# althonos/pyhmmer

Hardware: AMD Instinct MI355X
Metric: GCUPS (DP cells/s) + seqs/s for hmmsearch, Pfam-A vs proteome, 1/2/4/8 GPUs (higher is better)
Workload: dtype u8/i16 filters (MSV, Viterbi), f32 Forward/Backward

## Files before the change

pyhmmer_amd/csrc/p7x_msv.hip:

```cpp
#include <cstdlib>
#include <iterator>
#include "p7x_device.hpp"
#include "p7x_kernels.hpp"
#include "p7x_launch.hpp"

namespace p7x {

typedef short s2 __attribute__((ext_vector_type(2)));

__device__ __forceinline__ s2 as_s2(uint32_t u) { return __builtin_bit_cast(s2, u); }
__device__ __forceinline__ uint32_t as_u32(s2 v) { return __builtin_bit_cast(uint32_t, v); }
__device__ __forceinline__ s2 pk_max(s2 a, s2 b) { return __builtin_elementwise_max(a, b); }
__device__ __forceinline__ s2 pk_adds(s2 a, s2 b) { return __builtin_elementwise_add_sat(a, b); }
__device__ __forceinline__ s2 pk_subs(s2 a, s2 b) { return __builtin_elementwise_sub_sat(a, b); }
__device__ __forceinline__ s2 splat(int v) { s2 r; r.x = (short) v; r.y = (short) v; return r; }
__device__ __forceinline__ s2 swap_halves(s2 v) { return as_s2(__builtin_amdgcn_alignbit(as_u32(v), as_u32(v), 16)); }

typedef _Float16 h2 __attribute__((ext_vector_type(2)));
__device__ __forceinline__ h2 as_h2(s2 v) { return __builtin_bit_cast(h2, v); }
__device__ __forceinline__ s2 as_s2(h2 v) { return __builtin_bit_cast(s2, v); }
__device__ __forceinline__ s2 h_adds(s2 a, s2 b)
{
  const h2 z = { (_Float16) 0.0f, (_Float16) 0.0f }, o = { (_Float16) 1.0f, (_Float16) 1.0f };
  return as_s2(__builtin_elementwise_min(__builtin_elementwise_max(as_h2(a) + as_h2(b), z), o));
}
__device__ __forceinline__ s2 h_subs(s2 a, s2 b)
{
  const h2 z = { (_Float16) 0.0f, (_Float16) 0.0f }, o = { (_Float16) 1.0f, (_Float16) 1.0f };
  return as_s2(__builtin_elementwise_min(__builtin_elementwise_max(as_h2(a) - as_h2(b), z), o));
}
__device__ __forceinline__ s2 h_max(s2 a, s2 b) { return as_s2(__builtin_elementwise_maximum(as_h2(a), as_h2(b))); }
__device__ __forceinline__ s2 h_max3(s2 a, s2 b, s2 c)
{ return as_s2(__builtin_elementwise_maximum(__builtin_elementwise_maximum(as_h2(a), as_h2(b)), as_h2(c))); }
__device__ __forceinline__ s2 h_splat(int units)
{ const _Float16 x = (_Float16) ((float) units * (1.0f / 256.0f)); h2 r; r.x = x; r.y = x; return as_s2(r); }
__device__ __forceinline__ uint32_t h_of_i16_pair(uint32_t w)
{
  const int lo = max((int) (short) (w & 0xffffu), -512), hi = max((int) (short) (w >> 16), -512);
  return __builtin_bit_cast(uint32_t, __builtin_amdgcn_cvt_pkrtz((float) lo * (1.0f / 256.0f), (float) hi * (1.0f / 256.0f)));
}


constexpr int msv_stride_c(int R)
{
  int S = R + (R & 1);
  if (((S / 2) & 1) == 0) S += 2;
  return S;
}
constexpr int msv_lane_stride_c(int R, int K)
{
  if (K == 1) return msv_stride_c(R);
  int s = R + (R & 1);
  while (s % 64 != 2) s += 2;
  return s;
}
constexpr int msv_row_stride_c(int R, int K) { return K * msv_lane_stride_c(R, K); }
constexpr bool msv_uniform_c(int K) { return K >= 8; }
constexpr int msv_parities_c(int K) { return msv_uniform_c(K) ? 1 : 2; }
constexpr int msv_even_imm_c(int R, int K) { return K == 1 ? kTabRows * msv_row_stride_c(R, K) * 4 : 0; }
constexpr int msv_even_add_c(int R, int K) { return (K == 1 || msv_uniform_c(K)) ? 0 : kTabRows * msv_row_stride_c(R, K) * 4; }
constexpr int msv_block_c(int K) { return K == 1 ? 256 : 512; }
template <int K, bool H = false> __device__ __forceinline__ s2 target_max(s2 m)
{
  auto mx = [](s2 a, s2 b) { if constexpr (H) return h_max(a, b); else return pk_max(a, b); };
  if constexpr (K >= 2) m = mx(m, as_s2((uint32_t) __builtin_amdgcn_update_dpp(0, (int) as_u32(m), 0xB1, 0xf, 0xf, false)));
  if constexpr (K >= 4) m = mx(m, as_s2((uint32_t) __builtin_amdgcn_update_dpp(0, (int) as_u32(m), 0x4E, 0xf, 0xf, false)));
  if constexpr (K >= 8) m = mx(m, as_s2((uint32_t) __builtin_amdgcn_update_dpp(0, (int) as_u32(m), 0x141, 0xf, 0xf, false)));
  return m;
}
template <int K> __device__ __forceinline__ s2 carry_in(s2 last, s2 edge, int h)
{
  if constexpr (K == 1) return edge;
  const s2 up = as_s2((uint32_t) __builtin_amdgcn_update_dpp(0, (int) as_u32(last), 0x111, 0xf, 0xf, false));
  return h == 0 ? edge : up;
}

struct Chunk { uint2 e0, e1, e2, e3; };

template <int OFF>
__device__ __forceinline__ void lds_issue4(uint32_t addr, Chunk &c)
{
  asm volatile("ds_read_b64 %0, %4 offset:%5\n\t"
               "ds_read_b64 %1, %4 offset:%6\n\t"
               "ds_read_b64 %2, %4 offset:%7\n\t"
               "ds_read_b64 %3, %4 offset:%8"
               : "=&v"(c.e0), "=&v"(c.e1), "=&v"(c.e2), "=&v"(c.e3)
               : "v"(addr), "i"(OFF), "i"(OFF + 8), "i"(OFF + 16), "i"(OFF + 24));
}
template <int OFF>
__device__ __forceinline__ void lds_issue2(uint32_t addr, Chunk &c)
{
  asm volatile("ds_read_b64 %0, %2 offset:%3\n\t"
               "ds_read_b64 %1, %2 offset:%4"
               : "=&v"(c.e0), "=&v"(c.e1)
               : "v"(addr), "i"(OFF), "i"(OFF + 8));
}
template <int PENDING>
__device__ __forceinline__ void lds_wait4(Chunk &c)
{
  asm volatile("s_waitcnt lgkmcnt(%4)" : "+v"(c.e0), "+v"(c.e1), "+v"(c.e2), "+v"(c.e3) : "i"(PENDING));
}
template <int PENDING>
__device__ __forceinline__ void lds_wait2(Chunk &c)
{
  asm volatile("s_waitcnt lgkmcnt(%2)" : "+v"(c.e0), "+v"(c.e1) : "i"(PENDING));
}

template <int R, int TB, bool ODD, int T, int FAST = 0, bool U = false>
struct RowChunks {
  static_assert(!U || ODD, "the uniform row reads the register below: it is walked from the top register down");
  static_assert(R % 4 == 0, "a row is walked in chunks of 8 registers and a last one of 4: the register count must be a multiple of 4");
  static constexpr int NT = (R + 7) / 8;
  static constexpr int TBASE = TB;
  static constexpr int pairs(int t) { return (t == NT - 1 && (R % 8) != 0) ? 2 : 4; }

  template <int TT>
  static __device__ __forceinline__ void issue(uint32_t addr, Chunk &c)
  {
    if constexpr (pairs(TT) == 4) lds_issue4<TBASE + TT * 32>(addr, c); else lds_issue2<TBASE + TT * 32>(addr, c);
  }

  template <int JJ>
  static __device__ __forceinline__ void pair(s2 (&v)[R], const uint2 e, const s2 xB, const s2 carry, s2 &accA, s2 &accB)
  {
    if constexpr (U) {
      s2 pred = carry;
      if constexpr (JJ > 0) pred = v[2 * JJ - 1];
      const s2 d1 = as_s2(__builtin_amdgcn_alignbit(as_u32(v[2 * JJ + 1]), as_u32(v[2 * JJ]), 16));
      const s2 d0 = as_s2(__builtin_amdgcn_alignbit(as_u32(v[2 * JJ]), as_u32(pred), 16));
      if constexpr (FAST == 2) {
        v[2 * JJ + 1] = h_adds(d1, as_s2(e.y));
        v[2 * JJ] = h_adds(d0, as_s2(e.x));
        if constexpr (JJ & 1) { accB = h_max3(accB, v[2 * JJ], v[2 * JJ + 1]); asm volatile("" : "+v"(accB)); }
        else { accA = h_max3(accA, v[2 * JJ], v[2 * JJ + 1]); asm volatile("" : "+v"(accA)); }
      } else if constexpr (FAST == 1) {
        v[2 * JJ + 1] = pk_adds(d1, as_s2(e.y));
        v[2 * JJ] = pk_adds(d0, as_s2(e.x));
        accA = pk_max(accA, v[2 * JJ]);
        accB = pk_max(accB, v[2 * JJ + 1]);
        asm volatile("" : "+v"(accA), "+v"(accB));
      } else {
        v[2 * JJ + 1] = pk_max(d1, xB) + as_s2(e.y);
        accA = pk_max(accA, v[2 * JJ + 1]);
        v[2 * JJ] = pk_max(d0, xB) + as_s2(e.x);
        accB = pk_max(accB, v[2 * JJ]);
      }
    } else if constexpr (FAST == 2) {
      if constexpr (ODD) {
        v[2 * JJ + 1] = h_adds(v[2 * JJ], as_s2(e.y));
        s2 pred = carry;
        if constexpr (JJ > 0) pred = v[2 * JJ - 1];
        v[2 * JJ] = h_adds(pred, as_s2(e.x));
      } else {
        v[2 * JJ] = h_adds(v[2 * JJ], as_s2(e.x));
        v[2 * JJ + 1] = h_adds(v[2 * JJ + 1], as_s2(e.y));
      }
      if constexpr (JJ & 1) { accB = h_max3(accB, v[2 * JJ], v[2 * JJ + 1]); asm volatile("" : "+v"(accB)); }
      else { accA = h_max3(accA, v[2 * JJ], v[2 * JJ + 1]); asm volatile("" : "+v"(accA)); }
    } else if constexpr (FAST == 1) {
      if constexpr (ODD) {
        v[2 * JJ + 1] = pk_adds(v[2 * JJ], as_s2(e.y));
        s2 pred = carry;
        if constexpr (JJ > 0) pred = v[2 * JJ - 1];
        v[2 * JJ] = pk_adds(pred, as_s2(e.x));
      } else {
        v[2 * JJ] = pk_adds(v[2 * JJ], as_s2(e.x));
        v[2 * JJ + 1] = pk_adds(v[2 * JJ + 1], as_s2(e.y));
      }
      accA = pk_max(accA, v[2 * JJ]);
      accB = pk_max(accB, v[2 * JJ + 1]);
      asm volatile("" : "+v"(accA), "+v"(accB));
    } else if constexpr (ODD) {
      const s2 t1 = pk_max(v[2 * JJ], xB);
      v[2 * JJ + 1] = t1 + as_s2(e.y);
      accA = pk_max(accA, v[2 * JJ + 1]);
      s2 t0 = pk_max(carry, xB);
      if constexpr (JJ > 0) t0 = pk_max(v[2 * JJ - 1], xB);
      v[2 * JJ] = t0 + as_s2(e.x);
      accB = pk_max(accB, v[2 * JJ]);
    } else {
      v[2 * JJ] = pk_max(v[2 * JJ], xB) + as_s2(e.x);
      accA = pk_max(accA, v[2 * JJ]);
      v[2 * JJ + 1] = pk_max(v[2 * JJ + 1], xB) + as_s2(e.y);
      accB = pk_max(accB, v[2 * JJ + 1]);
    }
  }

  static __device__ __forceinline__ void run(s2 (&v)[R], uint32_t addr, Chunk &cur, Chunk &nxt, const s2 xB, const s2 carry, s2 &accA, s2 &accB)
  {
    constexpr bool last = ODD ? (T == 0) : (T == NT - 1);
    constexpr int TN = ODD ? T - 1 : T + 1;
    constexpr int np = pairs(T);
    if constexpr (!last) {
      issue<TN>(addr, nxt);
      if constexpr (np == 4) lds_wait4<pairs(TN)>(cur); else lds_wait2<pairs(TN)>(cur);
    } else {
      if constexpr (np == 4) lds_wait4<0>(cur); else lds_wait2<0>(cur);
    }
    if constexpr (ODD) {
      if constexpr (np == 4) {
        pair<4 * T + 3>(v, cur.e3, xB, carry, accA, accB);
        pair<4 * T + 2>(v, cur.e2, xB, carry, accA, accB);
      }
      pair<4 * T + 1>(v, cur.e1, xB, carry, accA, accB);
      pair<4 * T + 0>(v, cur.e0, xB, carry, accA, accB);
    } else {
      pair<4 * T + 0>(v, cur.e0, xB, carry, accA, accB);
      pair<4 * T + 1>(v, cur.e1, xB, carry, accA, accB);
      if constexpr (np == 4) {
        pair<4 * T + 2>(v, cur.e2, xB, carry, accA, accB);
        pair<4 * T + 3>(v, cur.e3, xB, carry, accA, accB);
      }
    }
    if constexpr (!last) RowChunks<R, TB, ODD, TN, FAST, U>::run(v, addr, nxt, cur, xB, carry, accA, accB);
  }
};

template <int R, int K, bool ODD>
__device__ __forceinline__ void msv_row(s2 (&v)[R], uint32_t addr, int h, s2 &xB, s2 &xJ, s2 &xEmax,
                                        const s2 basev, const s2 tecv, const s2 tjbmv, const s2 zerov)
{
  constexpr int NT = (R + 7) / 8;
  constexpr bool U = msv_uniform_c(K), DOWN = ODD || U;
  constexpr int T0 = DOWN ? NT - 1 : 0;
  constexpr int TB = DOWN ? 0 : msv_even_imm_c(R, K);
  const s2 carry = DOWN ? carry_in<K>(v[R - 1], xB, h) : xB;
  Chunk ca, cb;
  RowChunks<R, TB, DOWN, T0, 0, U>::template issue<T0>(addr, ca);
  s2 accA = splat(kNegPad), accB = accA;
  RowChunks<R, TB, DOWN, T0, 0, U>::run(v, addr, ca, cb, xB, carry, accA, accB);
  s2 m = pk_max(accA, accB);
  m = pk_max(m, swap_halves(m));
  m = target_max<K>(m);
  xEmax = pk_max(xEmax, m);
  m = m - tecv;
  xJ = pk_max(xJ, m);
  xB = pk_max(pk_max(basev, xJ) - tjbmv, zerov);
}

template <int K> struct MsvItem {
  int g, t, h;
  __device__ __forceinline__ MsvItem(int group, int part, int lane) : g(group), t(part * (64 / K) + lane / K), h(lane % K) {}
};

template <int R, int K>
__global__ void __launch_bounds__(msv_block_c(K)) msv_kernel(const ArgRef ref)
{
  extern __shared__ __attribute__((aligned(16))) uint32_t lds[];
  constexpr int S = msv_row_stride_c(R, K), Rs = msv_lane_stride_c(R, K), BLK = msv_block_c(K);
  const MsvArgs a = load_args<MsvArgs>(ref);
  const int nitems = (a.group_list ? *a.group_count : a.ngroups - a.group_first) * K;
  if (nitems <= 0 || *a.counter >= nitems) return;
  {
    constexpr int n4 = (msv_parities_c(K) * kTabRows * S) / 4;
    const uint4 *src = reinterpret_cast<const uint4 *>(a.tab);
    uint4 *dst = reinterpret_cast<uint4 *>(lds);
    for (int i = threadIdx.x; i < n4; i += BLK) dst[i] = src[i];
  }
  __syncthreads();

  const int lane = threadIdx.x & 63;
  const s2 basev = splat(a.base), tecv = splat(a.tec), zerov = splat(0);

  for (;;) {
    int item = 0;
    if (lane == 0) item = atomicAdd(a.counter, 1);
    item = __builtin_amdgcn_readfirstlane(item);
    if (item >= nitems) break;
    const int gi = item / K;
    const MsvItem<K> it(a.group_list ? __builtin_amdgcn_readfirstlane(a.group_list[gi]) : gi + a.group_first, item % K, lane);

    const int slot = it.g * 64 + it.t;
    const int L = a.slot_len[slot];
    const int nblk = a.grp_nblk[it.g];
    const uint4 *tp = a.tiles + a.grp_off[it.g] + it.t;
    const s2 tjbmv = splat((int) a.tjb_tab[L] + a.tbm);
    const uint32_t lane_col = (uint32_t) it.h * (uint32_t) (Rs * 4);

    s2 v[R];
#pragma unroll
    for (int j = 0; j < R; ++j) v[j] = zerov;
    s2 xJ = zerov, xEmax = zerov;
    s2 xB = pk_max(basev - tjbmv, zerov);

    uint4 cur = tp[0];
    for (int b = 0; b < nblk; ++b) {
      const uint4 nxt = (b + 1 < nblk) ? tp[(size_t) (b + 1) * 64] : cur;
      uint32_t w0 = cur.x, w1 = cur.y, w2 = cur.z, w3 = cur.w;
#pragma unroll 1
      for (int c = 0; c < 8; ++c) {
        const uint32_t x0 = w0 & 0xffu, x1 = (w0 >> 8) & 0xffu;
        w0 = __builtin_amdgcn_alignbit(w1, w0, 16); w1 = __builtin_amdgcn_alignbit(w2, w1, 16);
        w2 = __builtin_amdgcn_alignbit(w3, w2, 16); w3 >>= 16;
        msv_row<R, K, true >(v, x0 * (uint32_t) (S * 4) + lane_col, it.h, xB, xJ, xEmax, basev, tecv, tjbmv, zerov);
        msv_row<R, K, false>(v, x1 * (uint32_t) (S * 4) + lane_col + (uint32_t) msv_even_add_c(R, K), it.h, xB, xJ, xEmax, basev, tecv, tjbmv, zerov);
      }
      cur = nxt;
    }
    if (L > 0 && it.h == 0) {
      const int xe = xEmax.x;
      a.out_xJ[slot] = (xe >= 255 - a.bias) ? (int16_t) -1 : (int16_t) xJ.x;
    }
  }
}

template <int R, int K, bool H>
__device__ __forceinline__ void msv_fast_body(const MsvArgs &a, uint32_t *lds)
{
  constexpr int S = msv_row_stride_c(R, K), Rs = msv_lane_stride_c(R, K), BLK = msv_block_c(K);
  constexpr int MODE = H ? 2 : 1;
  const int nitems = (a.ngroups - a.group_first) * K;
  if (*a.counter >= nitems) return;
  {
    constexpr int n4 = (msv_parities_c(K) * kTabRows * S) / 4;
    const uint4 *src = reinterpret_cast<const uint4 *>(a.tab);
    uint4 *dst = reinterpret_cast<uint4 *>(lds);
    for (int i = threadIdx.x; i < n4; i += BLK) {
      uint4 w = src[i];
      if constexpr (H) { w.x = h_of_i16_pair(w.x); w.y = h_of_i16_pair(w.y); w.z = h_of_i16_pair(w.z); w.w = h_of_i16_pair(w.w); }
      dst[i] = w;
    }
  }
  __syncthreads();

  const int lane = threadIdx.x & 63;
  const s2 floorv = H ? as_s2(0u) : splat(-32768);
  constexpr int NT = (R + 7) / 8;
  auto mx = [](s2 x, s2 y) { if constexpr (H) return h_max(x, y); else return pk_max(x, y); };

  for (;;) {
    int item = 0;
    if (lane == 0) item = atomicAdd(a.counter, 1);
    item = __builtin_amdgcn_readfirstlane(item);
    if (item >= nitems) break;
    const MsvItem<K> it(item / K + a.group_first, item % K, lane);

    const int slot = it.g * 64 + it.t;
    const int L = a.slot_len[slot];
    const int nblk = a.grp_nblk[it.g];
    const uint2 *tp = reinterpret_cast<const uint2 *>(a.tiles + a.grp_off[it.g] + it.t);
    const int tjbm = (int) a.tjb_tab[L] + a.tbm;
    const uint32_t lane_col = (uint32_t) it.h * (uint32_t) (Rs * 4);

    s2 v[R];
#pragma unroll
    for (int j = 0; j < R; ++j) v[j] = floorv;
    int xJ = 0, xEmax = 0;
    int xB = max(a.base - tjbm, 0);
    const int F0 = xB - a.tec;
    const s2 Tv = H ? h_splat(tjbm + a.tec) : splat(tjbm + a.tec - 32768);
    s2 accA = floorv, accB = floorv;
    auto fold = [&](const s2 m2) -> int {
      int rel;
      if constexpr (H) { const h2 m = as_h2(m2); rel = (int) (256.0f * fmaxf((float) m.x, (float) m.y)); }
      else rel = max((int) m2.x, (int) m2.y) + 32768;
      const int xE = rel + xB;
      xEmax = max(xEmax, xE);
      xJ = max(xJ, xE - a.tec);
      return max(max(a.base, xJ) - tjbm, 0);
    };

    uint2 cur = tp[0];
    for (int hb = 0; hb < 2 * nblk; ++hb) {
      const uint2 nxt = (hb + 1 < 2 * nblk) ? tp[(size_t) ((hb + 1) >> 1) * 128 + ((hb + 1) & 1)] : cur;
      uint32_t w0 = cur.x, w1 = cur.y;
#pragma unroll 1
      for (int c = 0; c < 4; ++c) {
        const uint32_t x0 = w0 & 0xffu, x1 = (w0 >> 8) & 0xffu;
        w0 = __builtin_amdgcn_alignbit(w1, w0, 16); w1 >>= 16;
#pragma unroll
        for (int half = 0; half < 2; ++half) {
          Chunk ca, cb;
          if constexpr (msv_uniform_c(K)) {
            const uint32_t addr = (half == 0 ? x0 : x1) * (uint32_t) (S * 4) + lane_col;
            const s2 carry = carry_in<K>(v[R - 1], floorv, it.h);
            RowChunks<R, 0, true, NT - 1, MODE, true>::template issue<NT - 1>(addr, ca);
            RowChunks<R, 0, true, NT - 1, MODE, true>::run(v, addr, ca, cb, floorv, carry, accA, accB);
          } else if (half == 0) {
            const uint32_t addr = x0 * (uint32_t) (S * 4) + lane_col;
            const s2 carry = carry_in<K>(v[R - 1], floorv, it.h);
            RowChunks<R, 0, true, NT - 1, MODE>::template issue<NT - 1>(addr, ca);
            RowChunks<R, 0, true, NT - 1, MODE>::run(v, addr, ca, cb, floorv, carry, accA, accB);
          } else {
            const uint32_t addr = x1 * (uint32_t) (S * 4) + lane_col + (uint32_t) msv_even_add_c(R, K);
            RowChunks<R, msv_even_imm_c(R, K), false, 0, MODE>::template issue<0>(addr, ca);
            RowChunks<R, msv_even_imm_c(R, K), false, 0, MODE>::run(v, addr, ca, cb, floorv, floorv, accA, accB);
          }
          const s2 m2 = target_max<K, H>(mx(accA, accB));
          if (__builtin_expect(__any(as_u32(mx(m2, Tv)) != as_u32(Tv)), 0)) {
            asm volatile("; re-bias: the begin score moved" ::: "memory");
            const int xBn = fold(m2);
            const s2 dv = H ? h_splat(xBn - xB) : splat(xBn - xB);
#pragma unroll
            for (int j = 0; j < R; ++j) v[j] = H ? h_subs(v[j], dv) : pk_subs(v[j], dv);
            xB = xBn;
            accA = floorv; accB = floorv;
          }
        }
      }
      cur = nxt;
    }
    fold(target_max<K, H>(mx(accA, accB)));
    const bool ambiguous = (L > 0) && (xJ == F0) && !(xEmax >= 255 - a.bias);
    if (L > 0 && it.h == 0) a.out_xJ[slot] = (xEmax >= 255 - a.bias) ? (int16_t) -1 : (int16_t) xJ;
    if (__any(ambiguous) && lane == 0) { const int idx = atomicAdd(a.amb_count, 1); a.amb_groups[idx] = it.g; }
  }
}

constexpr int msv_min_blocks_c(int R, int K) { return K > 1 ? 2 : (R <= 92 ? 4 : (R <= 136 ? 3 : 2)); }

template <int R, int K, bool H>
__global__ void __launch_bounds__(msv_block_c(K), msv_min_blocks_c(R, K)) msv_fast_kernel(const ArgRef ref)
{
  extern __shared__ __attribute__((aligned(16))) uint32_t lds[];
  const MsvArgs a = load_args<MsvArgs>(ref);
  msv_fast_body<R, K, H>(a, lds);
}

#define P7X_TILES_TIER0(X) X(8, 1) X(12, 1) X(16, 1) X(20, 1) X(24, 1) X(28, 1) X(32, 1) X(36, 1) X(40, 1) X(44, 1) X(48, 1) X(52, 1) \
                           X(56, 1) X(60, 1) X(64, 1) X(68, 1) X(72, 1) X(76, 1) X(80, 1) X(84, 1) X(88, 1) X(92, 1)
#define P7X_TILES_TIER1(X) X(96, 1) X(100, 1) X(104, 1) X(108, 1) X(112, 1) X(116, 1) X(120, 1) X(124, 1) X(128, 1) X(132, 1) X(136, 1)
#define P7X_TILES_TIER2(X) X(140, 1) X(144, 1) X(148, 1) X(152, 1) X(156, 1) X(160, 1) X(176, 1) X(192, 1) X(208, 1) X(224, 1)
#define P7X_TILES_TIER3(X) X(120, 2) X(128, 2) X(136, 2) X(144, 2) X(152, 2) X(160, 2) X(168, 2) X(176, 2) X(184, 2) X(192, 2) X(200, 2) \
                           X(208, 2) X(216, 2) X(224, 2)
#define P7X_TILES_TIER4(X) X(120, 4) X(128, 4)
#define P7X_TILES_TIER5(X) X(64, 8) X(72, 8) X(80, 8) X(88, 8) X(96, 8) X(104, 8) X(112, 8) X(120, 8) X(128, 8)
constexpr int msv_tier_block_c(int T) { return T <= 2 ? 256 : 512; }
constexpr int msv_tier_min_blocks_c(int T) { return T == 0 ? 4 : (T == 1 ? 3 : 2); }

template <int TIER>
__global__ void __launch_bounds__(msv_tier_block_c(TIER), msv_tier_min_blocks_c(TIER)) msv_tier_kernel(const ArgRef ref)
{
  extern __shared__ __attribute__((aligned(16))) uint32_t lds[];
  const MsvArgs a = load_args<MsvArgs>(ref);
  const int R = __builtin_amdgcn_readfirstlane(a.R);
#define P7X_TILE(r, k) case r: msv_fast_body<r, k, true>(a, lds); break;
  if constexpr (TIER == 0) { switch (R) { P7X_TILES_TIER0(P7X_TILE) default: break; } }
  else if constexpr (TIER == 1) { switch (R) { P7X_TILES_TIER1(P7X_TILE) default: break; } }
  else if constexpr (TIER == 2) { switch (R) { P7X_TILES_TIER2(P7X_TILE) default: break; } }
  else if constexpr (TIER == 3) { switch (R) { P7X_TILES_TIER3(P7X_TILE) default: break; } }
  else if constexpr (TIER == 4) { switch (R) { P7X_TILES_TIER4(P7X_TILE) default: break; } }
  else { switch (R) { P7X_TILES_TIER5(P7X_TILE) default: break; } }
#undef P7X_TILE
}


#define P7X_R_ONLY(r, k) r,
static const int kRList[] = { P7X_TILES_TIER0(P7X_R_ONLY) P7X_TILES_TIER1(P7X_R_ONLY) P7X_TILES_TIER2(P7X_R_ONLY) };
static const int kRList2[] = { P7X_TILES_TIER3(P7X_R_ONLY) };
static const int kRList4[] = { P7X_TILES_TIER4(P7X_R_ONLY) };
static const int kRList8[] = { P7X_TILES_TIER5(P7X_R_ONLY) };
#undef P7X_R_ONLY
static bool msv_tile_exists(int R, int K)
{
  auto in = [R](const int *b, const int *e) { for (; b != e; ++b) if (*b == R) return true; return false; };
  switch (K) {
    case 1: return in(std::begin(kRList), std::end(kRList));
    case 2: return in(std::begin(kRList2), std::end(kRList2));
    case 4: return in(std::begin(kRList4), std::end(kRList4));
    case 8: return in(std::begin(kRList8), std::end(kRList8));
    default: return false;
  }
}

int msv_pick(int M, int *K)
{
  const int need = (M + 1) / 2 + 1;
  *K = 1;
  for (int r : kRList) if (r >= need) return r;
  *K = 2;
  for (int r : kRList2) if (2 * r >= need) return r;
  *K = 4;
  for (int r : kRList4) if (4 * r >= need) return r;
  *K = 8;
  if (debug_opt(OPT_MSV_K8) != 0)
    for (int r : kRList8) if (8 * r >= (M + 1) / 2) return r;
  *K = 0;
  return -1;
}

static int row_stride(int R, int K)
{
  int rs = R + (R & 1);
  if (K == 1) { if (((rs / 2) & 1) == 0) rs += 2; return rs; }
  while (rs % 64 != 2) rs += 2;
  return K * rs;
}
int msv_stride(int R, int K) { return row_stride(R, K); }
int msv_table_dwords(int R, int K) { return msv_parities_c(K) * kTabRows * row_stride(R, K); }

void msv_build_tables(const Profile &p, int R, int K, std::vector<uint32_t> &out)
{
  const int S = row_stride(R, K), Rs = S / K;
  out.assign((size_t) msv_table_dwords(R, K), 0);
  auto sval = [&](int x, int k) -> int {
    if (x >= p.Kp || k < 1 || k > p.M) return kNegPad;
    return (int) p.bias_b - (int) p.rb[(size_t) x * (p.M + 1) + k];
  };
  auto pack = [](int lo, int hi) -> uint32_t { return ((uint32_t) (uint16_t) (int16_t) lo) | ((uint32_t) (uint16_t) (int16_t) hi << 16); };
  if (msv_uniform_c(K)) {
    for (int x = 0; x < kTabRows; ++x)
      for (int h = 0; h < K; ++h)
        for (int r = 0; r < Rs; ++r) {
          const int j = h * R + r;
          out[(size_t) x * S + (size_t) h * Rs + r] = r < R ? pack(sval(x, 2 * j + 1), sval(x, 2 * j + 2)) : pack(kNegPad, kNegPad);
        }
    return;
  }
  for (int x = 0; x < kTabRows; ++x)
    for (int h = 0; h < K; ++h)
      for (int r = 0; r < Rs; ++r) {
        const bool live = r < R;
        const int j = h * R + r;
        out[((size_t) 0 * kTabRows + x) * S + (size_t) h * Rs + r] = live ? pack(sval(x, 2 * j - 1), sval(x, 2 * j)) : pack(kNegPad, kNegPad);
        out[((size_t) 1 * kTabRows + x) * S + (size_t) h * Rs + r] = live ? pack(sval(x, 2 * j), sval(x, 2 * j + 1)) : pack(kNegPad, kNegPad);
      }
}

template <int R, int K>
static int launch_RK(const ArgRun<MsvArgs> &main, const ArgRun<MsvArgs> *amb, int num_cu, hipStream_t st, bool amb_only = false)
{
  constexpr int BLK = msv_block_c(K);
  const size_t lds_bytes = (size_t) msv_parities_c(K) * kTabRows * msv_row_stride_c(R, K) * 4;
  int per_cu_exact = 0, per_cu_fast = 0, per_cu_half = 0;
  int pst = kernel_blocks_per_cu(&msv_kernel<R, K>, BLK, lds_bytes, &per_cu_exact);
  if (pst == P7X_OK) pst = kernel_blocks_per_cu(&msv_fast_kernel<R, K, false>, BLK, lds_bytes, &per_cu_fast);
  if (pst == P7X_OK) pst = kernel_blocks_per_cu(&msv_fast_kernel<R, K, true>, BLK, lds_bytes, &per_cu_half);
  if (pst != P7X_OK) return pst;
  if (amb_only) {
    hipLaunchKernelGGL((msv_kernel<R, K>), dim3(lane_grid(32, 32, amb->n), (unsigned) amb->n), dim3(BLK), lds_bytes, st, amb->ref());
    P7X_HIP(hipGetLastError());
    return P7X_OK;
  }
  constexpr int wpb = BLK / 64;
  long want = 1;
  for (int i = 0; i < main.n; ++i) want = std::max<long>(want, ((long) (main.at(i).ngroups - main.at(i).group_first) * K + wpb - 1) / wpb);
  if (amb == nullptr) {
    const unsigned gx = lane_grid_pull(want, (long) num_cu * per_cu_exact, main.n, debug_opt(OPT_MSV_LANE_BLOCKS) == 0);
    hipLaunchKernelGGL((msv_kernel<R, K>), dim3(gx, (unsigned) main.n), dim3(BLK), lds_bytes, st, main.ref());
    P7X_HIP(hipGetLastError());
    return P7X_OK;
  }
  const bool half = debug_opt(OPT_MSV_F16) != 0;
  int per_cu2 = half ? per_cu_half : per_cu_fast;
  const int cap = debug_opt(OPT_MSV_BLOCKS_PER_CU);
  if (cap > 0 && per_cu2 > cap) per_cu2 = cap;
  const unsigned gx2 = lane_grid_pull(want, (long) num_cu * per_cu2, main.n, debug_opt(OPT_MSV_LANE_BLOCKS) == 0);
  if (half) hipLaunchKernelGGL((msv_fast_kernel<R, K, true>), dim3(gx2, (unsigned) main.n), dim3(BLK), lds_bytes, st, main.ref());
  else hipLaunchKernelGGL((msv_fast_kernel<R, K, false>), dim3(gx2, (unsigned) main.n), dim3(BLK), lds_bytes, st, main.ref());
  P7X_HIP(hipGetLastError());
  hipLaunchKernelGGL((msv_kernel<R, K>), dim3(lane_grid(32, 32, amb->n), (unsigned) amb->n), dim3(BLK), lds_bytes, st, amb->ref());
  P7X_HIP(hipGetLastError());
  return P7X_OK;
}

static int msv_launch_impl(int R, int K, const ArgRun<MsvArgs> &main, const ArgRun<MsvArgs> *amb, int num_cu, hipStream_t st, bool amb_only);

int msv_launch(int R, int K, const ArgRun<MsvArgs> &main, const ArgRun<MsvArgs> *amb, int num_cu, hipStream_t st)
{ return msv_launch_impl(R, K, main, amb, num_cu, st, false); }

int msv_exact_launch(int R, int K, const ArgRun<MsvArgs> &amb, int num_cu, hipStream_t st)
{ return msv_launch_impl(R, K, amb, &amb, num_cu, st, true); }

int msv_tier(int R, int K)
{
  if (K == 1) return R <= 92 ? 0 : (R <= 136 ? 1 : 2);
  return K == 2 ? 3 : (K == 4 ? 4 : 5);
}

template <int TIER>
static int launch_tier(const ArgRun<MsvArgs> &main, int num_cu, hipStream_t st)
{
  constexpr int BLK = msv_tier_block_c(TIER), K = TIER <= 2 ? 1 : (TIER == 3 ? 2 : (TIER == 4 ? 4 : 8));
  int Rmax = 0;
  long want = 1;
  constexpr int wpb = BLK / 64;
  for (int i = 0; i < main.n; ++i) {
    const MsvArgs &a = main.at(i);
    if (msv_tier(a.R, K) != TIER || !msv_tile_exists(a.R, K)) { set_error("msv_tier_launch: a lane of another tier, or a register tile without a kernel"); return P7X_EINVAL; }
    Rmax = std::max(Rmax, a.R);
    want = std::max<long>(want, ((long) (a.ngroups - a.group_first) * K + wpb - 1) / wpb);
  }
  const size_t lds_bytes = (size_t) msv_table_dwords(Rmax, K) * 4;
  constexpr int Rtop = TIER == 0 ? 92 : (TIER == 1 ? 136 : (TIER >= 4 ? 128 : 224));
  int per_cu = 0;
  const int pst = kernel_blocks_per_cu(&msv_tier_kernel<TIER>, BLK, lds_bytes, &per_cu, (size_t) msv_table_dwords(Rtop, K) * 4);
  if (pst != P7X_OK) return pst;
  const unsigned gx = lane_grid_pull(want, (long) num_cu * per_cu, main.n, debug_opt(OPT_MSV_LANE_BLOCKS) == 0);
  hipLaunchKernelGGL((msv_tier_kernel<TIER>), dim3(gx, (unsigned) main.n), dim3(BLK), lds_bytes, st, main.ref());
  P7X_HIP(hipGetLastError());
  return P7X_OK;
}

int msv_tier_launch(int tier, const ArgRun<MsvArgs> &main, int num_cu, hipStream_t st)
{
  if (main.n <= 0) return P7X_OK;
  switch (tier) {
    case 0: return launch_tier<0>(main, num_cu, st);
    case 1: return launch_tier<1>(main, num_cu, st);
    case 2: return launch_tier<2>(main, num_cu, st);
    case 3: return launch_tier<3>(main, num_cu, st);
    case 4: return launch_tier<4>(main, num_cu, st);
    case 5: return launch_tier<5>(main, num_cu, st);
    default: set_error("msv_tier_launch: no such tier"); return P7X_EINVAL;
  }
}

static int msv_launch_impl(int R, int K, const ArgRun<MsvArgs> &main, const ArgRun<MsvArgs> *amb, int num_cu, hipStream_t st, bool amb_only)
{
  if (main.n <= 0) return P7X_OK;
  switch (K * 1000 + R) {
#define P7X_CASE(r, k) case k * 1000 + r: return launch_RK<r, k>(main, amb, num_cu, st, amb_only);
    P7X_TILES_TIER0(P7X_CASE) P7X_TILES_TIER1(P7X_CASE) P7X_TILES_TIER2(P7X_CASE) P7X_TILES_TIER3(P7X_CASE) P7X_TILES_TIER4(P7X_CASE) P7X_TILES_TIER5(P7X_CASE)
#undef P7X_CASE
    default: set_error("msv_launch: unsupported register tile"); return P7X_EINVAL;
  }
}

}
```

Before: 27100.

## Prefetch next residue row's LDS scores and trim MSV loop to wave max length

Issues the LDS loads for the second residue's first score chunk while the first residue's last chunk is still being consumed, so the two residue rows overlap instead of draining the queue between them. The per-group block loop is also bounded by the longest sequence in the wave rather than the group's padded block count, which skips padded residues. The register-pinning asm hints in the fp16 path now target the other accumulator. The read-ahead raises register pressure and adds chunk-buffer swapping logic, so it is limited to R <= 208.

```diff
diff --git a/pyhmmer_amd/csrc/p7x_msv.hip b/pyhmmer_amd/csrc/p7x_msv.hip
--- a/pyhmmer_amd/csrc/p7x_msv.hip
+++ b/pyhmmer_amd/csrc/p7x_msv.hip
@@ -3,6 +3,7 @@
 #include "p7x_device.hpp"
 #include "p7x_kernels.hpp"
 #include "p7x_launch.hpp"
+#include "p7x_wave.hpp"
 
 namespace p7x {
 
@@ -41,6 +42,7 @@
 }
 
 
+constexpr bool msv_read_ahead_c(int R) { return R <= 208; }
 constexpr int msv_stride_c(int R)
 {
   int S = R + (R & 1);
@@ -131,8 +133,8 @@
       if constexpr (FAST == 2) {
         v[2 * JJ + 1] = h_adds(d1, as_s2(e.y));
         v[2 * JJ] = h_adds(d0, as_s2(e.x));
-        if constexpr (JJ & 1) { accB = h_max3(accB, v[2 * JJ], v[2 * JJ + 1]); asm volatile("" : "+v"(accB)); }
-        else { accA = h_max3(accA, v[2 * JJ], v[2 * JJ + 1]); asm volatile("" : "+v"(accA)); }
+        if constexpr (JJ & 1) { accB = h_max3(accB, v[2 * JJ], v[2 * JJ + 1]); asm volatile("" : "+v"(accA)); }
+        else { accA = h_max3(accA, v[2 * JJ], v[2 * JJ + 1]); asm volatile("" : "+v"(accB)); }
       } else if constexpr (FAST == 1) {
         v[2 * JJ + 1] = pk_adds(d1, as_s2(e.y));
         v[2 * JJ] = pk_adds(d0, as_s2(e.x));
@@ -155,8 +157,8 @@
         v[2 * JJ] = h_adds(v[2 * JJ], as_s2(e.x));
         v[2 * JJ + 1] = h_adds(v[2 * JJ + 1], as_s2(e.y));
       }
-      if constexpr (JJ & 1) { accB = h_max3(accB, v[2 * JJ], v[2 * JJ + 1]); asm volatile("" : "+v"(accB)); }
-      else { accA = h_max3(accA, v[2 * JJ], v[2 * JJ + 1]); asm volatile("" : "+v"(accA)); }
+      if constexpr (JJ & 1) { accB = h_max3(accB, v[2 * JJ], v[2 * JJ + 1]); asm volatile("" : "+v"(accA)); }
+      else { accA = h_max3(accA, v[2 * JJ], v[2 * JJ + 1]); asm volatile("" : "+v"(accB)); }
     } else if constexpr (FAST == 1) {
       if constexpr (ODD) {
         v[2 * JJ + 1] = pk_adds(v[2 * JJ], as_s2(e.y));
@@ -186,7 +188,9 @@
     }
   }
 
-  static __device__ __forceinline__ void run(s2 (&v)[R], uint32_t addr, Chunk &cur, Chunk &nxt, const s2 xB, const s2 carry, s2 &accA, s2 &accB)
+  template <int NXOFF = 0, int NXP = 0>
+  static __device__ __forceinline__ void run(s2 (&v)[R], uint32_t addr, Chunk &cur, Chunk &nxt, const s2 xB, const s2 carry, s2 &accA, s2 &accB,
+                                             uint32_t naddr = 0)
   {
     constexpr bool last = ODD ? (T == 0) : (T == NT - 1);
     constexpr int TN = ODD ? T - 1 : T + 1;
@@ -194,6 +198,9 @@
     if constexpr (!last) {
       issue<TN>(addr, nxt);
       if constexpr (np == 4) lds_wait4<pairs(TN)>(cur); else lds_wait2<pairs(TN)>(cur);
+    } else if constexpr (NXP > 0) {
+      if constexpr (NXP == 4) lds_issue4<NXOFF>(naddr, nxt); else lds_issue2<NXOFF>(naddr, nxt);
+      if constexpr (np == 4) lds_wait4<NXP>(cur); else lds_wait2<NXP>(cur);
     } else {
       if constexpr (np == 4) lds_wait4<0>(cur); else lds_wait2<0>(cur);
     }
@@ -212,7 +219,7 @@
         pair<4 * T + 3>(v, cur.e3, xB, carry, accA, accB);
       }
     }
-    if constexpr (!last) RowChunks<R, TB, ODD, TN, FAST, U>::run(v, addr, nxt, cur, xB, carry, accA, accB);
+    if constexpr (!last) RowChunks<R, TB, ODD, TN, FAST, U>::template run<NXOFF, NXP>(v, addr, nxt, cur, xB, carry, accA, accB, naddr);
   }
 };
 
@@ -337,7 +344,8 @@
 
     const int slot = it.g * 64 + it.t;
     const int L = a.slot_len[slot];
-    const int nblk = a.grp_nblk[it.g];
+    const int npair = min((wave_max_i32(L) + 1) >> 1, 8 * a.grp_nblk[it.g]);
+    const int nhb = (npair + 3) >> 2;
     const uint2 *tp = reinterpret_cast<const uint2 *>(a.tiles + a.grp_off[it.g] + it.t);
     const int tjbm = (int) a.tjb_tab[L] + a.tbm;
     const uint32_t lane_col = (uint32_t) it.h * (uint32_t) (Rs * 4);
@@ -361,31 +369,17 @@
     };
 
     uint2 cur = tp[0];
-    for (int hb = 0; hb < 2 * nblk; ++hb) {
-      const uint2 nxt = (hb + 1 < 2 * nblk) ? tp[(size_t) ((hb + 1) >> 1) * 128 + ((hb + 1) & 1)] : cur;
+    for (int hb = 0; hb < nhb; ++hb) {
+      const uint2 nxt = (hb + 1 < nhb) ? tp[(size_t) ((hb + 1) >> 1) * 128 + ((hb + 1) & 1)] : cur;
+      const int nc = rfl(min(4, npair - 4 * hb));
       uint32_t w0 = cur.x, w1 = cur.y;
 #pragma unroll 1
-      for (int c = 0; c < 4; ++c) {
+      for (int c = 0; c < nc; ++c) {
         const uint32_t x0 = w0 & 0xffu, x1 = (w0 >> 8) & 0xffu;
         w0 = __builtin_amdgcn_alignbit(w1, w0, 16); w1 >>= 16;
-#pragma unroll
-        for (int half = 0; half < 2; ++half) {
-          Chunk ca, cb;
-          if constexpr (msv_uniform_c(K)) {
-            const uint32_t addr = (half == 0 ? x0 : x1) * (uint32_t) (S * 4) + lane_col;
-            const s2 carry = carry_in<K>(v[R - 1], floorv, it.h);
-            RowChunks<R, 0, true, NT - 1, MODE, true>::template issue<NT - 1>(addr, ca);
-            RowChunks<R, 0, true, NT - 1, MODE, true>::run(v, addr, ca, cb, floorv, carry, accA, accB);
-          } else if (half == 0) {
-            const uint32_t addr = x0 * (uint32_t) (S * 4) + lane_col;
-            const s2 carry = carry_in<K>(v[R - 1], floorv, it.h);
-            RowChunks<R, 0, true, NT - 1, MODE>::template issue<NT - 1>(addr, ca);
-            RowChunks<R, 0, true, NT - 1, MODE>::run(v, addr, ca, cb, floorv, carry, accA, accB);
-          } else {
-            const uint32_t addr = x1 * (uint32_t) (S * 4) + lane_col + (uint32_t) msv_even_add_c(R, K);
-            RowChunks<R, msv_even_imm_c(R, K), false, 0, MODE>::template issue<0>(addr, ca);
-            RowChunks<R, msv_even_imm_c(R, K), false, 0, MODE>::run(v, addr, ca, cb, floorv, floorv, accA, accB);
-          }
+        Chunk ca, cb;
+        constexpr bool FREE_B = ((NT - 1) % 2) == 0, AHEAD = msv_read_ahead_c(R);
+        auto rebias = [&]() {
           const s2 m2 = target_max<K, H>(mx(accA, accB));
           if (__builtin_expect(__any(as_u32(mx(m2, Tv)) != as_u32(Tv)), 0)) {
             asm volatile("; re-bias: the begin score moved" ::: "memory");
@@ -396,6 +390,32 @@
             xB = xBn;
             accA = floorv; accB = floorv;
           }
+        };
+        if constexpr (msv_uniform_c(K)) {
+          using Row = RowChunks<R, 0, true, NT - 1, MODE, true>;
+          const uint32_t addr0 = x0 * (uint32_t) (S * 4) + lane_col, addr1 = x1 * (uint32_t) (S * 4) + lane_col;
+          const s2 carry0 = carry_in<K>(v[R - 1], floorv, it.h);
+          Row::template issue<NT - 1>(addr0, ca);
+          Row::template run<(NT - 1) * 32, AHEAD ? Row::pairs(NT - 1) : 0>(v, addr0, ca, cb, floorv, carry0, accA, accB, addr1);
+          rebias();
+          const s2 carry1 = carry_in<K>(v[R - 1], floorv, it.h);
+          if constexpr (!AHEAD) { Row::template issue<NT - 1>(addr1, ca); Row::run(v, addr1, ca, cb, floorv, carry1, accA, accB); }
+          else if constexpr (FREE_B) Row::run(v, addr1, cb, ca, floorv, carry1, accA, accB);
+          else Row::run(v, addr1, ca, cb, floorv, carry1, accA, accB);
+          rebias();
+        } else {
+          using Odd = RowChunks<R, 0, true, NT - 1, MODE>;
+          using Even = RowChunks<R, msv_even_imm_c(R, K), false, 0, MODE>;
+          const uint32_t addr0 = x0 * (uint32_t) (S * 4) + lane_col;
+          const uint32_t addr1 = x1 * (uint32_t) (S * 4) + lane_col + (uint32_t) msv_even_add_c(R, K);
+          const s2 carry = carry_in<K>(v[R - 1], floorv, it.h);
+          Odd::template issue<NT - 1>(addr0, ca);
+          Odd::template run<Even::TBASE, AHEAD ? Even::pairs(0) : 0>(v, addr0, ca, cb, floorv, carry, accA, accB, addr1);
+          rebias();
+          if constexpr (!AHEAD) { Even::template issue<0>(addr1, ca); Even::run(v, addr1, ca, cb, floorv, floorv, accA, accB); }
+          else if constexpr (FREE_B) Even::run(v, addr1, cb, ca, floorv, floorv, accA, accB);
+          else Even::run(v, addr1, ca, cb, floorv, floorv, accA, accB);
+          rebias();
         }
       }
       cur = nxt;
```

After: 27210, median of 2. No clear change (+0.4%).
